# posgraph/coupe.optical_flow_based_deep_video_stabilization

Hardware: AMD Instinct MI355X
Metric: stabilised frame-pairs/sec @512x512 (higher is better)
Workload: dtype f32; 1 GPU; batch=8 512x512x27 frame stacks per GPU: FlowNetS-pyramid forward (5 flows) + flow resize/scale + tf_warp at 512x512; batch_per_gpu=8, height=512, width=512, cin=27, all_gather=False, vgg16_trunk=False, st_warp=none, plan_flags=0, plan_batch=0, full=False

## Files before the change

### coupe/optical_flow_based_deep_video_stabilization_amd/_lib.py

```python
from __future__ import annotations

import ctypes as C
import os

from . import build as _build

c_float_p = C.POINTER(C.c_float)
c_int32_p = C.POINTER(C.c_int32)


class VstabTensor(C.Structure):
    _fields_ = [("name", C.c_char_p), ("data", c_float_p), ("ndim", C.c_int32), ("shape", C.c_int32 * 4)]


class VstabWsEntry(C.Structure):
    _fields_ = [("name", C.c_char * 24), ("offset_bytes", C.c_int64), ("n", C.c_int32), ("h", C.c_int32),
                ("w", C.c_int32), ("c", C.c_int32), ("c_stride", C.c_int32)]


EXPORTS = {
    "vstab_create": (C.c_int, [C.POINTER(C.c_void_p), C.c_int]),
    "vstab_destroy": (None, [C.c_void_p]),
    "vstab_last_error": (C.c_char_p, [C.c_void_p]),
    "vstab_version": (C.c_char_p, []),
    "vstab_load_weights": (C.c_int, [C.c_void_p, C.POINTER(VstabTensor), C.c_int]),
    "vstab_workspace_bytes": (C.c_size_t, [C.c_int] * 4),
    "vstab_workspace_layout": (C.c_int, [C.c_int] * 4 + [C.POINTER(VstabWsEntry), C.c_int]),
    "vstab_workspace_layout_ctx": (C.c_int, [C.c_void_p] + [C.c_int] * 4 + [C.POINTER(VstabWsEntry), C.c_int]),
    "vstab_set_plan_batch": (C.c_int, [C.c_void_p, C.c_int]),
    "vstab_set_plan_flags": (C.c_int, [C.c_void_p, C.c_uint]),
    "vstab_workspace_bytes_ctx": (C.c_size_t, [C.c_void_p] + [C.c_int] * 4),
    "vstab_flownets_forward": (C.c_int, [C.c_void_p, C.c_void_p] + [C.c_int] * 4 + [C.c_void_p] * 5 +
                               [C.c_void_p, C.c_size_t, C.c_void_p]),
    "vstab_flow_resize_scale": (C.c_int, [C.c_void_p] + [C.c_int] * 3 + [C.c_void_p] + [C.c_int] * 4 + [C.c_void_p]),
    "vstab_resize_bilinear": (C.c_int, [C.c_void_p] + [C.c_int] * 4 + [C.c_void_p] + [C.c_int] * 2 + [C.c_void_p]),
    "vstab_resize_bilinear_slice3": (C.c_int, [C.c_void_p] + [C.c_int] * 5 + [C.c_void_p] + [C.c_int] * 2 + [C.c_void_p]),
    "vstab_warp_flow": (C.c_int, [C.c_void_p] * 3 + [C.c_int] * 4 + [C.c_void_p]),
    "vstab_selftest_div_const": (C.c_int, [C.c_float, C.c_uint, C.c_ulonglong, C.c_void_p, C.c_void_p]),
    "vstab_flow_glue_warp": (C.c_int, [C.c_void_p] + [C.c_int] * 3 + [C.c_void_p] * 3 + [C.c_int] * 5 + [C.c_void_p]),
    "vstab_stabilise_originalsize": (C.c_int, [C.c_void_p, C.c_void_p] + [C.c_int] * 4 + [C.c_void_p] + [C.c_int] * 2 + [C.c_void_p] * 8 +
                                     [C.c_size_t, C.c_void_p]),
    "vstab_trace_ranges": (C.c_int, [C.c_int]),
    "vstab_hbm_profile_enable": (C.c_int, [C.c_int]),
    "vstab_hbm_profile_read": (C.c_int, [C.c_int, C.POINTER(C.c_double), C.POINTER(C.c_int), C.POINTER(C.c_double)]),
    "vstab_get_pixel_value": (C.c_int, [C.c_void_p] * 4 + [C.c_int] * 6 + [C.c_void_p]),
# ... 144 lines not shown
```

### coupe/optical_flow_based_deep_video_stabilization_amd/build.py

```python
from __future__ import annotations

import os
import shutil
import subprocess

HERE = os.path.dirname(os.path.abspath(__file__))
CSRC = os.path.join(HERE, "csrc")
LIB = os.path.join(HERE, "libvstab_hip.so")
SOURCES = ("conv_mfma.hip", "conv_rowwin.hip", "conv_skinny.hip", "tap_panel.hip", "wino_gemm_stream.hip", "flow_ops.hip", "sampler_ops.hip", "sampler3d_ops.hip", "nldf_ops.hip", "clip_ops.hip", "train_ops.hip", "wgrad_mfma.hip", "winograd_ops.hip", "homography_ops.hip", "pack.cpp", "conv_desc.cpp", "api.cpp", "flownet_plan.cpp", "flownet_forward.cpp", "vgg_api.cpp", "nldf_api.cpp", "train_api.cpp")
HEADERS = ("vstab_internal.h", "api_internal.h", "conv_desc.h", "flownet_plan.h", "hbm_profile.h", "tile3.h", "st_axis.h", "conv_kloop_gfx950.inc", os.path.join("..", "..", "..", "include", "vstab.h"))
FLAGS = ["--offload-arch=gfx950", "-O3", "-std=c++17", "-ffp-contract=off", "-fPIC", "-fvisibility=hidden",
         "-Wall", "-Wno-unused-result"]


def hipcc() -> str:
    for c in (os.environ.get("HIPCC"), shutil.which("hipcc"), "/opt/rocm/bin/hipcc"):
        if c and os.path.exists(c):
            return c
    raise RuntimeError("hipcc not found (set HIPCC)")


STAMP = os.path.join(HERE, "libvstab_hip.so.srchash")


# ... 100 lines not shown
```

### coupe/optical_flow_based_deep_video_stabilization_amd/csrc/api.cpp

```cpp
#include <cmath>
#include <cstdlib>
#include <new>
#include <vector>

#include "api_internal.h"

using namespace vstab;

static thread_local std::string g_last_error;

int fail(vstab_ctx *ctx, int code, const char *fmt, ...)
{
    char buf[512];
    va_list ap;
    va_start(ap, fmt);
    vsnprintf(buf, sizeof buf, fmt, ap);
    va_end(ap);
    g_last_error = buf;
    if (ctx) { std::lock_guard<std::mutex> g(ctx->err_mu); ctx->err = buf; }
    return code;
}

void adopt_last_error(vstab_ctx *ctx)
{
// ... 58 lines not shown

extern "C" const char *vstab_version(void) { return "vstab-hip 0.1 (gfx950)"; }

extern "C" const char *vstab_last_error(const vstab_ctx *ctx) { return ctx ? ctx->err.c_str() : g_last_error.c_str(); }

extern "C" int vstab_create(vstab_ctx **out, int device)
{
    if (!out) return fail(nullptr, VSTAB_E_STATE, "vstab_create: out is NULL");
    *out = nullptr;
    int n = 0;
    HIP_TRY(nullptr, hipGetDeviceCount(&n));
    if (device < 0 || device >= n) return fail(nullptr, VSTAB_E_HIP, "vstab_create: device %d of %d", device, n);
    HIP_TRY(nullptr, hipSetDevice(device));
    HIP_TRY(nullptr, conv_set_attributes());
    HIP_TRY(nullptr, rowwin_set_attributes());
    HIP_TRY(nullptr, tap_panel_set_attributes());
    HIP_TRY(nullptr, wino_gemm_stream_set_attributes());
    vstab_ctx *c = new (std::nothrow) vstab_ctx();
    if (!c) return fail(nullptr, VSTAB_E_NOMEM, "vstab_create: out of host memory");
    c->device = device;
    *out = c;
    return VSTAB_OK;
}

extern "C" void vstab_destroy(vstab_ctx *ctx)
{
    if (!ctx) return;
    if (ctx->dev_weights) (void)hipFree(ctx->dev_weights);
    for (hipEvent_t e : ctx->prof_ev) (void)hipEventDestroy(e);
    if (ctx->vgg_weights) (void)hipFree(ctx->vgg_weights);
// ... 560 lines not shown
```

### coupe/optical_flow_based_deep_video_stabilization_amd/csrc/api_internal.h

```cpp
#pragma once
#include <cstdarg>
#include <cstdio>
#include <cstring>
#include <initializer_list>
#include <mutex>
#include <string>
#include <vector>

#include "../../../include/vstab.h"
#include "vstab_internal.h"

struct vstab_ctx {
    int device = 0;
    bool loaded = false;
    int cin = 0;
    std::string err;
    std::mutex err_mu;
    float *dev_weights = nullptr;
    size_t dev_weight_floats = 0;
    size_t enc_w[10], enc_b[10];
    size_t enc0_rw = 0;
    size_t zero_b = 0;
    size_t wino_w[10] = {0};
    size_t dec_w[4], dec_b[4];
    size_t wdec_w[4] = {0};
    size_t pred_w[4], pred_b[4];
    size_t tab_wp, tab_b, pred2_b;
    vstab::UpflowW up[4];
    int plan_batch = 0;
    unsigned plan_flags = 0;
    bool prof = false;
    std::vector<hipEvent_t> prof_ev;
    int prof_forwards = 0;
    double prof_flops[15] = {0};
    double prof_flops_direct[15] = {0};
    const char *prof_kernel[15] = {nullptr};
// ... 50 lines not shown
```

### coupe/optical_flow_based_deep_video_stabilization_amd/csrc/flownet_forward.cpp

```cpp
#include <cmath>
#include <cstdlib>

#include "flownet_plan.h"

using namespace vstab;

static const char *UP_NAME[4] = {"upsample6_5", "upsample5_4", "upsample4_3", "upsample3_2"};

extern "C" int vstab_load_weights(vstab_ctx *ctx, const vstab_tensor *t, int count)
{
    if (!ctx) return fail(nullptr, VSTAB_E_STATE, "vstab_load_weights: ctx is NULL");
    if (!t || count <= 0) return fail(ctx, VSTAB_E_WEIGHTS, "vstab_load_weights: no tensors");
    const vstab_tensor *w1 = find(t, count, "1/W_conv2d");
    if (!w1 || w1->ndim != 4) return fail(ctx, VSTAB_E_WEIGHTS, "missing variable 1/W_conv2d");
    const int cin = w1->shape[2];
    if (cin < 1 || cin > 4096) return fail(ctx, VSTAB_E_WEIGHTS, "1/W_conv2d: bad Cin %d", cin);

    std::vector<float> host;
    auto reserve = [&](size_t n) { size_t o = (host.size() + 63) / 64 * 64; host.resize(o + n, 0.f); return o; };
    std::vector<double> scale;
    auto need = [&](const std::string &name, std::initializer_list<int> s) -> const vstab_tensor * {
        const vstab_tensor *x = find(t, count, name);
        return shape_is(x, s) ? x : nullptr;
    };
// ... 14 lines not shown
        const int npad = padded_cols(e.cout);
        const KLayout L = conv_layout(e.k, e.k, ci, cs_in);
        scale.assign(npad, 1.0);
        ctx->enc_b[i] = reserve(npad);
        fold_bn(b->data, beta->data, mean->data, var->data, e.cout, npad, scale.data(), host.data() + ctx->enc_b[i]);
        ctx->enc_w[i] = reserve((size_t)L.ktiles() * npad * 32);
        pack_conv(W->data, scale.data(), e.k, e.k, ci, cs_in, e.cout, npad, L, host.data() + ctx->enc_w[i]);
        if (e.k == 3 && e.s == 1 && (ci & 31) == 0 && (e.cout & 127) == 0) {
            ctx->wino_w[i] = reserve((size_t)16 * (ci / 32) * e.cout * 32);
            pack_winograd(W->data, scale.data(), ci, e.cout, e.cout, host.data() + ctx->wino_w[i]);
        }
        if (i == 0) {
            const int lead = rowwin_lead(-e.p, cin), segp = rowwin_segp(-e.p, e.k, cin);
            ctx->enc0_rw = reserve((size_t)e.k * (segp / 32) * npad * 32);
            pack_conv_rowwin(W->data, scale.data(), e.k, e.k, cin, e.cout, npad, lead, segp, host.data() + ctx->enc0_rw);
        }
    }
    for (int l = 0; l < 4; ++l) {
        const Layer &d = dec_layer(l);
        const std::string n = d.name;
        const int co = d.cout, ci = d.cin, cs = in_buf(d).cs;
        NEED(W, n + "/W_deconv2d", 4, 4, co, ci)
        NEED(b, n + "/b_deconv2d", co)
        NEED(beta, n + "_bn/beta", co)
        NEED(mean, n + "_bn/moving_mean", co)
        NEED(var, n + "_bn/moving_variance", co)
        const int npad = padded_cols(co);
        scale.assign(npad, 1.0);
        ctx->dec_b[l] = reserve(npad);
        fold_bn(b->data, beta->data, mean->data, var->data, co, npad, scale.data(), host.data() + ctx->dec_b[l]);
// ... 85 lines not shown
        }
        const int rc = forward_chunk(ctx, feats + (size_t)b0 * H * W * Cin, bc, H, W, Cin,
                                     pf6 + (size_t)b0 * eh[9] * ew[9] * 2, pf5 + (size_t)b0 * eh[7] * ew[7] * 2,
                                     pf4 + (size_t)b0 * eh[5] * ew[5] * 2, pf3 + (size_t)b0 * eh[3] * ew[3] * 2,
                                     pf2 + (size_t)b0 * (H - 2) * (W - 2) * 2, workspace, workspace_bytes, stream_, (tail && all_fused) ? &t : nullptr);
        if (rc != VSTAB_OK) return rc;
        if (tail && all_fused && !t.fused) {
            if (b0 != 0) return fail(ctx, VSTAB_E_ALIGN, "stabilise: chunk %d of the batch misses the fused tail's alignment", b0 / chunk);
            all_fused = false;
        }
    }
    if (tail) tail->fused = all_fused;
    return VSTAB_OK;
}

static int forward_chunk(vstab_ctx *ctx, const float *feats, int B, int H, int W, int Cin, float *pf6, float *pf5,
                         float *pf4, float *pf3, float *pf2, void *workspace, size_t workspace_bytes, void *stream_, FusedTail *tail)
{
    Plan pl;
    const PlanPin pin = pin_of(ctx);
    if (!make_plan(B, H, W, Cin, pl, &pin)) return fail(ctx, VSTAB_E_SHAPE, "forward: unsupported problem %dx%dx%dx%d", B, H, W, Cin);
    if (workspace_bytes < pl.total) return fail(ctx, VSTAB_E_NOMEM, "forward: workspace %zu < %zu bytes", workspace_bytes, pl.total);
    if (((uintptr_t)workspace & 255) != 0) return fail(ctx, VSTAB_E_ALIGN, "forward: workspace must be 256-byte aligned");
    if (((uintptr_t)feats & 15) || ((uintptr_t)pf6 & 7) || ((uintptr_t)pf5 & 7) || ((uintptr_t)pf4 & 7) ||
        ((uintptr_t)pf3 & 7) || ((uintptr_t)pf2 & 7))
        return fail(ctx, VSTAB_E_ALIGN, "forward: feats must be 16-byte and flows 8-byte aligned");
    hipStream_t stream = (hipStream_t)stream_;
    char *ws = (char *)workspace;
    auto buf = [&](int b) { return (float *)(ws + pl.off[b]); };
    const float *dw = ctx->dev_weights;
// ... 27 lines not shown
            if (i >= 10 && i < 14 && pl.wdec[i - 10]) dmac = (double)B * p.Ho * p.Wo * 4.0 * NET[i].cin * p.N;
            ctx->prof_flops_direct[i] += 2.0 * dmac;
        }
    }
#define PROF_NAME(slot, name) do { if (ev) ctx->prof_kernel[slot] = (name); } while (0)
#define EV_A(slot) (ev ? ev[2 * (slot)] : nullptr)
#define EV_B(slot) (ev ? ev[2 * (slot) + 1] : nullptr)

    static const char *const HEAD_RANGE[4] = {"predict_flow6+upsample6_5", "predict_flow5+upsample5_4", "predict_flow4+upsample4_3", "predict_flow3+upsample3_2"};
    TraceRange whole_range("flownetS_pyramid");
    for (int i = 0; i < 10; ++i) {
        const Layer &e = NET[i];
        TraceRange layer_range(e.name);
        ConvParams p = pl.cp[i];
        if (i == 0) {
            RowWinParams r{};
            r.in = feats; r.out = buf(B_CONV1); r.wpk = dw + ctx->enc0_rw; r.bias = dw + ctx->enc_b[0];
            const long long in_bytes = (long long)B * H * W * Cin * 4;
            r.in_bytes = (unsigned)std::min<long long>(in_bytes, 0xFFFFFFFFLL);
            r.B = B; r.Hi = H; r.Wi = W; r.Cs_in = Cin; r.KH = e.k;
            r.SEGP = rowwin_segp(-e.p, e.k, Cin);
            r.s_in = e.s; r.off_y = -e.p;
            r.e_off = -e.p * Cin - rowwin_lead(-e.p, Cin);
            r.w_a = ((r.e_off % 4) + 4) % 4;
            r.MB = rowwin_mb(B, p.Ho, p.Wo);
            r.WLEN = round_up(r.s_in * Cin * (64 * r.MB - 1) + r.w_a + r.SEGP, 4);
            r.Ho = p.Ho; r.Wo = p.Wo; r.Cs_out = p.Cs_out; r.c_off = 0; r.N = p.N; r.Npad = p.Npad; r.act = 1;
            if (in_bytes < 0x80000000LL && rowwin_applicable(r)) {
                if (!tickets_cleared) { r.clear_words = tickets; r.clear_n = SKINNY_MAX_TILES; tickets_cleared = true; }
                const int rem = p.Wo % 128;
                if (r.MB == 2 && p.Wo > 128 && rem >= 1 && rem <= 64) {
                    RowWinParams t = r;
                    r.ntile_x = p.Wo / 128;
                    t.MB = 1; t.ox_base = r.ntile_x * 128; t.ntile_x = 1; t.clear_n = 0;
                    t.WLEN = round_up(t.s_in * Cin * 63 + t.w_a + t.SEGP, 4);
                    if (rowwin_applicable(t)) {
                        HIP_TRY(ctx, launch_conv_rowwin(r, stream, EV_A(0), nullptr));
                        HIP_TRY(ctx, launch_conv_rowwin(t, stream, nullptr, EV_B(0)));
                        PROF_NAME(0, "conv_rowwin_kernel<7, 2> + <4, 1> tail");
                        continue;
                    }
                    r.ntile_x = 0;
                }
                HIP_TRY(ctx, launch_conv_rowwin(r, stream, EV_A(0), EV_B(0)));
                PROF_NAME(0, r.MB == 2 ? "conv_rowwin_kernel<7, 2>" : "conv_rowwin_kernel<4, 1>");
                continue;
            }
        }
        if (!tickets_cleared) { HIP_TRY(ctx, hipMemsetAsync(tickets, 0, pl.bytes[B_TICKETS], stream)); tickets_cleared = true; }
        if (pl.wino[i]) {
            ConvParams q = pl.wcp[i];
            const int cin_i = e.cin;
            HIP_TRY(ctx, launch_wino_input(buf(e.in), B, pl.eh[i], pl.ew[i], in_buf(e).cs, 0, cin_i, buf(B_WINO_V), stream));
            q.in = buf(B_WINO_V); q.out = buf(B_WINO_M);
            q.wpk = dw + ctx->wino_w[i]; q.bias = dw + ctx->zero_b; q.partial = buf(B_PARTIAL);
            const int T_i = ((pl.eh[i] + 1) / 2) * ((pl.ew[i] + 1) / 2);
            const int P_i = wino_gemm_stream_positions(B, T_i, cin_i, e.cout);
            if (P_i > 0) {
                HIP_TRY(ctx, launch_wino_gemm_stream(q.in, q.wpk, q.out, B, T_i, cin_i, e.cout, P_i, stream, EV_A(i), EV_B(i)));
                PROF_NAME(i, "wino_gemm_stream_kernel");
            } else {
                HIP_TRY(ctx, launch_conv(q, pl.wtile[i], true, stream, EV_A(i), EV_B(i)));
// ... 236 lines not shown
```

### coupe/optical_flow_based_deep_video_stabilization_amd/csrc/flownet_plan.cpp

```cpp
#include <cmath>
#include <cstdlib>
#include <memory>
#include <new>

#include "flownet_plan.h"

using namespace vstab;

bool level_sizes(int H, int W, int *eh, int *ew)
{
    int h = H, w = W;
    for (int i = 0; i < 10; ++i) {
        h = (h + 2 * NET[i].p - NET[i].k) / NET[i].s + 1;
        w = (w + 2 * NET[i].p - NET[i].k) / NET[i].s + 1;
        if (h < 1 || w < 1) return false;
        eh[i] = h; ew[i] = w;
    }
    for (int l = 0; l < 4; ++l)
        if ((eh[LVL_ENC[l + 1]] + 1) / 2 != eh[LVL_ENC[l]] || (ew[LVL_ENC[l + 1]] + 1) / 2 != ew[LVL_ENC[l]]) return false;
    return H >= 3 && W >= 3;
}

static double split_cost_us(long long tiles, int KT, int ks, double slab_bytes, int BN, int BM, int *ks_eff_out)
{
// ... 153 lines not shown
        const Layer &e = NET[i];
        ConvParams &p = pl.cp[i];
        const int cin = i == 0 ? Cin : e.cin, cs_in = i == 0 ? Cin : in_buf(e).cs;
        p = conv_desc_plain(B, i == 0 ? H : pl.eh[i - 1], i == 0 ? W : pl.ew[i - 1], cin, cs_in, e.k, e.s, e.p, pl.eh[i], pl.ew[i], e.cout,
                            padded_cols(e.cout), out_buf(e).cs, e.c_off, 1);
        pl.tile[i] = default_tile(e.cout);
        pl.vec4[i] = (p.Cs_in % 4 == 0) && (p.SEG % 4 == 0);
        if (ref) { pl.tile[i] = ref->tile[i]; pl.skinny[i] = ref->skinny[i]; p.ksplit = ref->cp[i].ksplit; }
        else {
            pl.tile[i] = choose_tile_split(p, pl.tile[i], pl.vec4[i]);
            pl.skinny[i] = i > 0 && choose_skinny(p, pl.vec4[i], flags);
            if (pl.skinny[i]) pl.tile[i] = TILE_SKINNY;
        }
        if (p.ksplit > 1) partial_floats = std::max(partial_floats, (size_t)p.ksplit * p.Mmax * p.Npad);
    }
    size_t wino_v = 0, wino_m = 0;
    for (int i = 0; i < 10; ++i) {
        pl.wino[i] = false;
        const Layer &e = NET[i];
        if (e.k != 3 || e.s != 1 || e.p != 1 || pl.skinny[i]) continue;
        if (ref ? !ref->wino[i] : (in_buf(e).cs != e.cin || !wino_applies(B, pl.eh[i], pl.ew[i], e.cin, e.cout))) continue;
        const int TH = (pl.eh[i] + 1) / 2, TW = (pl.ew[i] + 1) / 2;
        pl.wcp[i] = conv_desc_wino_gemm(B, pl.eh[i], pl.ew[i], e.cin, e.cout);
        {
            const long long t128 = 16LL * ((pl.wcp[i].Mmax + 127) / 128) * (e.cout / 128);
            pl.wtile[i] = t128 >= 1024 ? TILE_128x128 : TILE_128x64;
        }
        wino_v = std::max(wino_v, (size_t)B * 16 * TH * TW * e.cin);
        wino_m = std::max(wino_m, (size_t)B * 16 * TH * TW * e.cout);
        pl.wino[i] = true;
// ... 87 lines not shown
    if (chunk < 1 || !make_plan(chunk, H, W, Cin, pl)) { fail(nullptr, VSTAB_E_SHAPE, "unsupported problem %dx%dx%dx%d", B, H, W, Cin); return 0; }
    return pl.total;
}

extern "C" int vstab_set_plan_batch(vstab_ctx *ctx, int batch)
{
    if (!ctx) return fail(nullptr, VSTAB_E_STATE, "set_plan_batch: ctx is NULL");
    if (batch < 0) return fail(ctx, VSTAB_E_SHAPE, "set_plan_batch: batch must be >= 0 (0 = plan for the batch of each call)");
    ctx->plan_batch = batch;
    return VSTAB_OK;
}

extern "C" int vstab_set_plan_flags(vstab_ctx *ctx, unsigned flags)
{
    if (!ctx) return fail(nullptr, VSTAB_E_STATE, "set_plan_flags: ctx is NULL");
    if (flags & ~(unsigned)(VSTAB_PLAN_NO_SKINNY | VSTAB_PLAN_NO_DUAL | VSTAB_PLAN_NO_TAIL | VSTAB_PLAN_NO_WDEC | VSTAB_PLAN_FORCE_WDEC)) return fail(ctx, VSTAB_E_SHAPE, "set_plan_flags: unknown flag bits 0x%x", flags);
    ctx->plan_flags = flags;
    return VSTAB_OK;
}

extern "C" size_t vstab_workspace_bytes_ctx(const vstab_ctx *ctx, int B, int H, int W, int Cin)
{
    Plan pl;
    const PlanPin pin = pin_of(ctx);
    if (pin.batch > 0 && B > pin.batch) { fail(nullptr, VSTAB_E_SHAPE, "batch %d exceeds the pinned plan batch %d", B, pin.batch); return 0; }
    const int chunk = B >= 1 ? chunk_size(pin, B, H, W, Cin) : 0;
    if (chunk < 1 || !make_plan(chunk, H, W, Cin, pl, &pin)) { fail(nullptr, VSTAB_E_SHAPE, "unsupported problem %dx%dx%dx%d", B, H, W, Cin); return 0; }
    return pl.total;
}

static int workspace_layout_of(const PlanPin *pin, int chunk, int H, int W, int Cin, vstab_ws_entry *entries, int max_entries)
// ... 116 lines not shown
```

### coupe/optical_flow_based_deep_video_stabilization_amd/csrc/flownet_plan.h

```cpp
#pragma once
#include "api_internal.h"
#include "conv_desc.h"

enum Buf { B_CONV1, B_CONCAT2, B_CONV3, B_CONCAT3, B_CONV4, B_CONCAT4, B_CONV5, B_CONCAT5, B_CONV6, B_CONV6_1, B_T,
           B_T6, B_T5, B_T4, B_T3, B_TICKETS, B_PARTIAL, B_WINO_V, B_WINO_M, N_BUF };
static_assert(B_PARTIAL == N_BUF - 3 && B_WINO_V == N_BUF - 2 && B_WINO_M == N_BUF - 1, "plan-dependent buffers must come last");

struct BufSpec { const char *name; int level, c, cs; };
constexpr BufSpec BUFS[N_BUF] = {
    {"conv1", 0, 64, 64},         {"concat2", 1, 194, 196},   {"conv3", 2, 256, 256},     {"concat3", 3, 386, 388},
    {"conv4", 4, 512, 512},       {"concat4", 5, 770, 772},   {"conv5", 6, 512, 512},     {"concat5", 7, 1026, 1028},
    {"conv6", 8, 1024, 1024},     {"conv6_1", 9, 1024, 1024}, {"pf2_taps", 1, 32, 32},    {"pf6_taps", 9, 32, 32},
    {"pf5_taps", 7, 32, 32},      {"pf4_taps", 5, 32, 32},    {"pf3_taps", 3, 32, 32},    {"tickets", -1, 0, 0},
    {"splitk", -1, 0, 0},         {"winograd_in", -1, 0, 0},  {"winograd_out", -1, 0, 0}};

enum LayerKind { L_CONV, L_DECONV, L_TAPS };
struct Layer { const char *name; LayerKind kind; int k, s, p, cin, cout, in, out, c_off; };
constexpr int N_LAYER = 19;
constexpr Layer NET[N_LAYER] = {
    {"conv1", L_CONV, 7, 2, 3, 0, 64, -1, B_CONV1, 0},              {"conv2", L_CONV, 5, 2, 2, 64, 128, B_CONV1, B_CONCAT2, 0},
    {"conv3", L_CONV, 5, 2, 2, 128, 256, B_CONCAT2, B_CONV3, 0},    {"conv3_1", L_CONV, 3, 1, 1, 256, 256, B_CONV3, B_CONCAT3, 0},
    {"conv4", L_CONV, 3, 2, 1, 256, 512, B_CONCAT3, B_CONV4, 0},    {"conv4_1", L_CONV, 3, 1, 1, 512, 512, B_CONV4, B_CONCAT4, 0},
    {"conv5", L_CONV, 3, 2, 1, 512, 512, B_CONCAT4, B_CONV5, 0},    {"conv5_1", L_CONV, 3, 1, 1, 512, 512, B_CONV5, B_CONCAT5, 0},
    {"conv6", L_CONV, 3, 2, 1, 512, 1024, B_CONCAT5, B_CONV6, 0},   {"conv6_1", L_CONV, 3, 1, 1, 1024, 1024, B_CONV6, B_CONV6_1, 0},
// ... 22 lines not shown
    for (int b = 0; b < N_BUF; ++b)
        if (BUFS[b].cs < BUFS[b].c || (BUFS[b].cs & 3)) return false;
    return NET[14].in == dec_layer(3).out;
}
static_assert(net_is_consistent(), "NET and BUFS disagree");

struct Plan {
    int B, H, W, Cin;
    int eh[10], ew[10];
    size_t off[N_BUF];
    size_t bytes[N_BUF];
    size_t total;
    vstab::ConvParams cp[N_LAYER];
    vstab::ConvTile tile[N_LAYER];
    bool vec4[N_LAYER];
    bool skinny[N_LAYER];
    bool wino[10];
    vstab::ConvParams wcp[10];
    vstab::ConvTile wtile[10];
    bool wdec[4];
    vstab::ConvParams wdcp[4];
    vstab::ConvTile wdtile[4];
    vstab::WdecGeom wdg[4];
    int buf_h(int b) const { return BUFS[b].level < 0 ? 0 : eh[BUFS[b].level]; }
    int buf_w(int b) const { return BUFS[b].level < 0 ? 0 : ew[BUFS[b].level]; }
};

struct PlanPin { int batch = 0; unsigned flags = 0; };
inline PlanPin pin_of(const vstab_ctx *ctx)
{
// ... 9 lines not shown
```

### coupe/optical_flow_based_deep_video_stabilization_amd/csrc/pack.cpp

```cpp
#include <cmath>
#include <cstring>

#include "vstab_internal.h"

namespace vstab {

KLayout klayout_run(int kh, int kw, int cs_in)
{
    KLayout L{kh, 1, kw * cs_in, round_up(kw * cs_in, 32), 0};
    return L;
}
KLayout klayout_tap(int kh, int kw, int cin, int cs_in)
{
    KLayout L{kh, kw, cin, round_up(cin, 32), cs_in};
    return L;
}
KLayout klayout_deconv(int cs_in) { return klayout_run(2, 2, cs_in); }

void fold_bn(const float *b, const float *beta, const float *mean, const float *var, int cout, int npad,
             double *scale, float *bias_out)
{
    for (int n = 0; n < npad; ++n) {
        double s = 1.0, bb = 0.0;
        if (n < cout) {
// ... 43 lines not shown
}

void pack_conv_rowwin(const float *W, const double *scale, int kh, int kw, int cin, int cout, int npad, int lead,
                      int segp, float *wpk)
{
    const int kpr = segp / 32;
    std::memset(wpk, 0, sizeof(float) * (size_t)kh * kpr * npad * 32);
    for (int ky = 0; ky < kh; ++ky)
        for (int kx = 0; kx < kw; ++kx)
            for (int ci = 0; ci < cin; ++ci) {
                const int k = lead + kx * cin + ci;
                float *row = wpk + ((size_t)ky * kpr + k / 32) * npad * 32;
                for (int n = 0; n < cout; ++n)
                    row[(size_t)n * 32 + perm_rowwin(k & 31)] =
                        (float)((double)W[(((size_t)ky * kw + kx) * cin + ci) * cout + n] * scale[n]);
            }
}

void pack_deconv(const float *W, const double *scale, int cin, int cs_in, int cout, int npad, float *wpk)
{
    const KLayout L = klayout_deconv(cs_in);
    const size_t phase_floats = (size_t)L.ktiles() * npad * 32;
    for (int py = 0; py < 2; ++py)
        for (int px = 0; px < 2; ++px) {
            pack_generic(L, cs_in, cin, 2, cout, npad,
                         [&](int t, int bx, int ci, int n) {
                             const int ky = 3 - py - 2 * t, kx = 3 - px - 2 * bx;
                             return (float)((double)W[(((size_t)ky * 4 + kx) * cout + n) * cin + ci] * scale[n]);
                         },
                         wpk + (size_t)(py * 2 + px) * phase_floats);
// ... 148 lines not shown
```

### coupe/optical_flow_based_deep_video_stabilization_amd/csrc/vstab_internal.h

```cpp
#pragma once
#include <hip/hip_runtime.h>
#include <stddef.h>
#include <stdint.h>

namespace vstab {

inline int round_up_c(int a, int b) { return (a + b - 1) / b * b; }

#ifdef __HIPCC__
#define VSTAB_HD __host__ __device__
#else
#define VSTAB_HD
#endif
VSTAB_HD inline void xcd_remap_calc(unsigned Nx, unsigned Ny, unsigned Nz, unsigned lin, unsigned &bx, unsigned &by, unsigned &bz)
{
    const unsigned T = Nx * Ny * Nz;
    const unsigned q = T >> 3, r = T & 7u, c = lin & 7u, idx = lin >> 3;
    const unsigned nl = (c < r ? c * (q + 1) : r * (q + 1) + (c - r) * q) + idx;
    unsigned t2;
    if ((Ny & (Ny - 1)) == 0) { const unsigned s = 31u - (unsigned)__builtin_clz(Ny); by = nl & (Ny - 1); t2 = nl >> s; }
    else { by = nl % Ny; t2 = nl / Ny; }
    if ((Nz & (Nz - 1)) == 0) { const unsigned s = 31u - (unsigned)__builtin_clz(Nz); bz = t2 & (Nz - 1); bx = t2 >> s; }
    else { bz = t2 % Nz; bx = t2 / Nz; }
}
// ... 131 lines not shown
    int asm_loop;
    int stream_rows;
    unsigned *clear_words;
    int clear_n;
    int ox_base, ntile_x;
};
inline int rowwin_mb(int B, int Ho, int Wo) { return (long long)B * Ho * ((Wo + 127) / 128) < 512 ? 1 : 2; }
bool rowwin_applicable(const RowWinParams &p);
hipError_t rowwin_set_attributes();
hipError_t launch_conv_rowwin(const RowWinParams &p, hipStream_t stream, hipEvent_t ev_start = nullptr,
                              hipEvent_t ev_stop = nullptr);
inline int rowwin_lead(int off_x, int cs) { return ((off_x * cs) % 2 != 0) ? 1 : 0; }
inline int rowwin_segp(int off_x, int kw, int cs) { return round_up_c(rowwin_lead(off_x, cs) + kw * cs, 32); }
void pack_conv_rowwin(const float *W, const double *scale, int kh, int kw, int cin, int cout, int npad,
                      int lead, int segp, float *wpk);

hipError_t launch_wino_outgrad(const float *dy, int B, int H, int W, int Cs, int c_off, int C, float *dM, hipStream_t stream);
hipError_t launch_wino_filter_grad(const float *dU, int cin, int cout, float *dW, hipStream_t stream);
int wino_gemm_stream_positions(int B, int T, int cin, int cout);
hipError_t launch_wino_gemm_stream(const float *V, const float *wpk, float *M, int B, int T, int cin, int cout, int P, hipStream_t stream,
                                   hipEvent_t ev_start = nullptr, hipEvent_t ev_stop = nullptr);
hipError_t wino_gemm_stream_set_attributes();
hipError_t launch_wino_input(const float *x, int B, int H, int W, int Cs, int c_off, int C, float *V, hipStream_t stream,
                             bool pos_major = false);
hipError_t launch_wino_weights(const float *W, int cin, int cout, int transpose, float *Wt, hipStream_t stream);
hipError_t launch_wino_output(const float *M, int B, int Ho, int Wo, int C, const float *bias, int act, float *out, int Cs_out, int c_off,
                              hipStream_t stream);

struct WdecGeom {
    int NTy, NTx;
// ... 260 lines not shown
```

### include/vstab.h

```cpp
#ifndef VSTAB_H
#define VSTAB_H

#include <stddef.h>
#include <stdint.h>

#ifdef __cplusplus
extern "C" {
#endif

#define VSTAB_OK          0
#define VSTAB_E_SHAPE    -1
#define VSTAB_E_ALIGN    -2
#define VSTAB_E_HIP      -3
#define VSTAB_E_NOMEM    -4
#define VSTAB_E_WEIGHTS  -5
#define VSTAB_E_STATE    -6

#if defined(__GNUC__)
#define VSTAB_API __attribute__((visibility("default")))
#else
#define VSTAB_API
#endif

typedef struct vstab_ctx vstab_ctx;
// ... 202 lines not shown
VSTAB_API int vstab_flow_mean_fill(const float *flow, int B, int h, int w, float *out, void *stream);

VSTAB_API size_t vstab_homography_workspace_bytes(int B, int H, int W, int K);
VSTAB_API int vstab_homography_fit(const float *flow, int B, int H, int W, int K, unsigned seed, double thresh, int refine,
                                   int stride, double *Hout, int32_t *inliers, void *workspace, size_t workspace_bytes,
                                   void *stream);
VSTAB_API int vstab_warp_perspective_u8(const uint8_t *src, int B, int sh, int sw, const double *Hm, uint8_t *dst, int oh, int ow,
                                        void *stream);


#define VSTAB_PLAN_NO_SKINNY 1u
#define VSTAB_PLAN_NO_DUAL 2u
#define VSTAB_PLAN_NO_TAIL 4u
#define VSTAB_PLAN_NO_WDEC 8u
#define VSTAB_PLAN_FORCE_WDEC 16u
VSTAB_API int vstab_set_plan_flags(vstab_ctx *ctx, unsigned flags);

VSTAB_API int vstab_profile_enable(vstab_ctx *ctx, int enable);
VSTAB_API int vstab_profile_reset(vstab_ctx *ctx);
VSTAB_API int vstab_profile_read(vstab_ctx *ctx, double *ms_sum15, double *flops15, int *n_forwards);
VSTAB_API int vstab_profile_read_direct(vstab_ctx *ctx, double *flops15);
VSTAB_API int vstab_profile_kernel_name(vstab_ctx *ctx, int slot, char *buf, int cap);

VSTAB_API int vstab_selftest_div_const(float d, unsigned first_bits, unsigned long long count, unsigned long long *bad_count_dev,
                                       void *stream);

VSTAB_API int vstab_trace_ranges(int on);

VSTAB_API int vstab_hbm_profile_enable(int mode);
VSTAB_API int vstab_hbm_profile_read(int slot, double *ms_sum, int *launches, double *alg_bytes_sum);

// ... 17 lines not shown
```

Baseline: 2850 frame-pairs/s.

## Run conv1 on bf16 MFMA with three-way split for fp32-level accuracy

Adds a new conv1 row-window kernel that splits fp32 inputs and weights into three bf16 components (hi/mid/lo) and computes the product with six bf16 MFMA passes, replacing the fp32 rowwin path when cout is 64. The input split is done in LDS per kernel row, and weights are pre-split at load time. The aim is to use the much higher bf16 matrix throughput for the first, large-spatial convolution while keeping accuracy close to fp32. It adds split arithmetic, three times the LDS planes and extra MFMA passes, and it can be turned off with a new plan flag.

```diff
diff --git a/coupe/optical_flow_based_deep_video_stabilization_amd/_lib.py b/coupe/optical_flow_based_deep_video_stabilization_amd/_lib.py
--- a/coupe/optical_flow_based_deep_video_stabilization_amd/_lib.py
+++ b/coupe/optical_flow_based_deep_video_stabilization_amd/_lib.py
@@ -29,6 +29,7 @@
     "vstab_workspace_layout_ctx": (C.c_int, [C.c_void_p] + [C.c_int] * 4 + [C.POINTER(VstabWsEntry), C.c_int]),
     "vstab_set_plan_batch": (C.c_int, [C.c_void_p, C.c_int]),
     "vstab_set_plan_flags": (C.c_int, [C.c_void_p, C.c_uint]),
+    "vstab_conv1_forward": (C.c_int, [C.c_void_p, C.c_void_p] + [C.c_int] * 4 + [C.c_void_p, C.c_int, C.c_int, C.c_void_p]),
     "vstab_workspace_bytes_ctx": (C.c_size_t, [C.c_void_p] + [C.c_int] * 4),
     "vstab_flownets_forward": (C.c_int, [C.c_void_p, C.c_void_p] + [C.c_int] * 4 + [C.c_void_p] * 5 +
                                [C.c_void_p, C.c_size_t, C.c_void_p]),
diff --git a/coupe/optical_flow_based_deep_video_stabilization_amd/build.py b/coupe/optical_flow_based_deep_video_stabilization_amd/build.py
--- a/coupe/optical_flow_based_deep_video_stabilization_amd/build.py
+++ b/coupe/optical_flow_based_deep_video_stabilization_amd/build.py
@@ -7,7 +7,7 @@
 HERE = os.path.dirname(os.path.abspath(__file__))
 CSRC = os.path.join(HERE, "csrc")
 LIB = os.path.join(HERE, "libvstab_hip.so")
-SOURCES = ("conv_mfma.hip", "conv_rowwin.hip", "conv_skinny.hip", "tap_panel.hip", "wino_gemm_stream.hip", "flow_ops.hip", "sampler_ops.hip", "sampler3d_ops.hip", "nldf_ops.hip", "clip_ops.hip", "train_ops.hip", "wgrad_mfma.hip", "winograd_ops.hip", "homography_ops.hip", "pack.cpp", "conv_desc.cpp", "api.cpp", "flownet_plan.cpp", "flownet_forward.cpp", "vgg_api.cpp", "nldf_api.cpp", "train_api.cpp")
+SOURCES = ("conv_mfma.hip", "conv_rowwin.hip", "conv1_bf16x3.hip", "conv_skinny.hip", "tap_panel.hip", "wino_gemm_stream.hip", "flow_ops.hip", "sampler_ops.hip", "sampler3d_ops.hip", "nldf_ops.hip", "clip_ops.hip", "train_ops.hip", "wgrad_mfma.hip", "winograd_ops.hip", "homography_ops.hip", "pack.cpp", "conv_desc.cpp", "api.cpp", "flownet_plan.cpp", "flownet_forward.cpp", "vgg_api.cpp", "nldf_api.cpp", "train_api.cpp")
 HEADERS = ("vstab_internal.h", "api_internal.h", "conv_desc.h", "flownet_plan.h", "hbm_profile.h", "tile3.h", "st_axis.h", "conv_kloop_gfx950.inc", os.path.join("..", "..", "..", "include", "vstab.h"))
 FLAGS = ["--offload-arch=gfx950", "-O3", "-std=c++17", "-ffp-contract=off", "-fPIC", "-fvisibility=hidden",
          "-Wall", "-Wno-unused-result"]
diff --git a/coupe/optical_flow_based_deep_video_stabilization_amd/csrc/api.cpp b/coupe/optical_flow_based_deep_video_stabilization_amd/csrc/api.cpp
--- a/coupe/optical_flow_based_deep_video_stabilization_amd/csrc/api.cpp
+++ b/coupe/optical_flow_based_deep_video_stabilization_amd/csrc/api.cpp
@@ -96,6 +96,7 @@
     HIP_TRY(nullptr, hipSetDevice(device));
     HIP_TRY(nullptr, conv_set_attributes());
     HIP_TRY(nullptr, rowwin_set_attributes());
+    HIP_TRY(nullptr, conv1_bf16x3_set_attributes());
     HIP_TRY(nullptr, tap_panel_set_attributes());
     HIP_TRY(nullptr, wino_gemm_stream_set_attributes());
     vstab_ctx *c = new (std::nothrow) vstab_ctx();
diff --git a/coupe/optical_flow_based_deep_video_stabilization_amd/csrc/api_internal.h b/coupe/optical_flow_based_deep_video_stabilization_amd/csrc/api_internal.h
--- a/coupe/optical_flow_based_deep_video_stabilization_amd/csrc/api_internal.h
+++ b/coupe/optical_flow_based_deep_video_stabilization_amd/csrc/api_internal.h
@@ -20,6 +20,7 @@
     size_t dev_weight_floats = 0;
     size_t enc_w[10], enc_b[10];
     size_t enc0_rw = 0;
+    size_t enc0_b3 = 0;
     size_t zero_b = 0;
     size_t wino_w[10] = {0};
     size_t dec_w[4], dec_b[4];
diff --git a/coupe/optical_flow_based_deep_video_stabilization_amd/csrc/conv1_bf16x3.hip b/coupe/optical_flow_based_deep_video_stabilization_amd/csrc/conv1_bf16x3.hip
--- /dev/null
+++ b/coupe/optical_flow_based_deep_video_stabilization_amd/csrc/conv1_bf16x3.hip
@@ -0,0 +1,220 @@
+#include <hip/hip_ext.h>
+
+#include "vstab_internal.h"
+
+namespace vstab {
+
+typedef float f32x4 __attribute__((ext_vector_type(4)));
+typedef float f32x16 __attribute__((ext_vector_type(16)));
+typedef unsigned u32x2 __attribute__((ext_vector_type(2)));
+typedef unsigned u32x4 __attribute__((ext_vector_type(4)));
+typedef __bf16 bf16x4 __attribute__((ext_vector_type(4)));
+typedef __bf16 bf16x8 __attribute__((ext_vector_type(8)));
+
+template <int NWIN4, int MB>
+__global__ __launch_bounds__(256) void conv1_bf16x3_kernel(const RowWinParams p)
+{
+    extern __shared__ __attribute__((aligned(16))) char smem[];
+    unsigned *planes = reinterpret_cast<unsigned *>(smem);
+
+    const int tid = threadIdx.x, lane = tid & 63, wave = tid >> 6;
+    const int wm = wave >> 1, wn = wave & 1;
+    const int li = lane & 31, lh = lane >> 5;
+    unsigned bx_, by_, bz_;
+    xcd_remap(bx_, by_, bz_);
+    if (p.clear_n > 0 && blockIdx.x == 0 && blockIdx.y == 0 && blockIdx.z == 0)
+        for (int i = tid; i < p.clear_n; i += 256) p.clear_words[i] = 0u;
+    const int oy = (int)bx_;
+    const int ox0 = p.ox_base + (int)by_ * (64 * MB), n = (int)bz_;
+    const int pix_step = p.s_in * p.Cs_in;
+    const int row_floats = p.Wi * p.Cs_in;
+    const int g0 = pix_step * ox0 + p.e_off - p.w_a;
+
+    const __amdgpu_buffer_rsrc_t rin = __builtin_amdgcn_make_buffer_rsrc(const_cast<float *>(p.in), 0, p.in_bytes, 0x00020000);
+    const unsigned OOB = 0xC0000000u;
+
+    f32x4 wv[NWIN4];
+    auto load_window = [&](int ky) {
+        const int iy = oy * p.s_in + p.off_y + ky;
+        const bool yok = (unsigned)iy < (unsigned)p.Hi;
+        const int rowbase = ((n * p.Hi + iy) * p.Wi) * p.Cs_in;
+#pragma unroll
+        for (int j = 0; j < NWIN4; ++j) {
+            const int c4 = tid + 256 * j;
+            const int g = g0 + 4 * c4;
+            const bool ok = yok && g >= 0 && g < row_floats && 4 * c4 < p.WLEN;
+            const unsigned off = ok ? (unsigned)(rowbase + g) * 4u : OOB;
+            wv[j] = __builtin_bit_cast(f32x4, __builtin_amdgcn_raw_buffer_load_b128(rin, off, 0, 0));
+        }
+    };
+    const int plane_w = p.WLEN >> 1;
+    auto split_store = [&]() {
+#pragma unroll
+        for (int j = 0; j < NWIN4; ++j) {
+            const int c4 = tid + 256 * j;
+            if (4 * c4 < p.WLEN) {
+                bf16x4 h, m, l;
+#pragma unroll
+                for (int e = 0; e < 4; ++e) {
+                    const float x = wv[j][e];
+                    h[e] = (__bf16)x;
+                    const float r1 = x - (float)h[e];
+                    m[e] = (__bf16)r1;
+                    const float r2 = r1 - (float)m[e];
+                    l[e] = (__bf16)r2;
+                }
+                *reinterpret_cast<u32x2 *>(planes + 2 * c4) = __builtin_bit_cast(u32x2, h);
+                *reinterpret_cast<u32x2 *>(planes + plane_w + 2 * c4) = __builtin_bit_cast(u32x2, m);
+                *reinterpret_cast<u32x2 *>(planes + 2 * plane_w + 2 * c4) = __builtin_bit_cast(u32x2, l);
+            }
+        }
+    };
+
+    const int KG = p.SEGP >> 4;
+    const int NG = p.KH * KG;
+    const unsigned *bbase = reinterpret_cast<const unsigned *>(p.wpk) + (wn * 32 + li) * 8 + lh * 4;
+    auto load_b = [&](u32x4 (&b)[3], int G) {
+        const unsigned *s = bbase + (long long)(G < NG ? G : NG - 1) * (3 * 512);
+#pragma unroll
+        for (int q = 0; q < 3; ++q) b[q] = *reinterpret_cast<const u32x4 *>(s + q * 512);
+    };
+    const int a_w0 = (pix_step * (wm * 32 * MB + li) + p.w_a + 8 * lh) >> 1;
+    const int a_w1 = a_w0 + ((pix_step * 32) >> 1);
+    auto load_a = [&](u32x4 (&a)[3 * MB], int g) {
+#pragma unroll
+        for (int mb = 0; mb < MB; ++mb)
+#pragma unroll
+            for (int q = 0; q < 3; ++q) {
+                const unsigned *s = planes + q * plane_w + (mb ? a_w1 : a_w0) + 8 * g;
+                u32x4 v;
+                v.x = s[0]; v.y = s[1]; v.z = s[2]; v.w = s[3];
+                a[mb * 3 + q] = v;
+            }
+    };
+
+    f32x16 acc[MB];
+#pragma unroll
+    for (int a = 0; a < MB; ++a)
+#pragma unroll
+        for (int r = 0; r < 16; ++r) acc[a][r] = 0.f;
+
+    auto mma = [&](const u32x4 (&a)[3 * MB], const u32x4 (&b)[3]) {
+        constexpr int PA[6] = {2, 1, 0, 1, 0, 0}, PB[6] = {0, 1, 2, 0, 1, 0};
+#pragma unroll
+        for (int t = 0; t < 6; ++t)
+#pragma unroll
+            for (int mb = 0; mb < MB; ++mb)
+                acc[mb] = __builtin_amdgcn_mfma_f32_32x32x16_bf16(__builtin_bit_cast(bf16x8, a[mb * 3 + PA[t]]),
+                                                                  __builtin_bit_cast(bf16x8, b[PB[t]]), acc[mb], 0, 0, 0);
+    };
+
+    u32x4 a0[3 * MB], a1[3 * MB], b0[3], b1[3];
+    load_window(0);
+    load_b(b0, 0);
+    split_store();
+    __syncthreads();
+    int G = 0;
+    for (int ky = 0; ky < p.KH; ++ky) {
+        const bool more = ky + 1 < p.KH;
+        if (more) load_window(ky + 1);
+        load_a(a0, 0);
+        __builtin_amdgcn_sched_barrier(0);
+        for (int g = 0; g < KG; g += 2, G += 2) {
+            load_a(a1, g + 1);
+            load_b(b1, G + 1);
+            __builtin_amdgcn_sched_barrier(0);
+            mma(a0, b0);
+            __builtin_amdgcn_sched_barrier(0);
+            if (g + 2 < KG) load_a(a0, g + 2);
+            load_b(b0, G + 2);
+            __builtin_amdgcn_sched_barrier(0);
+            mma(a1, b1);
+            __builtin_amdgcn_sched_barrier(0);
+        }
+        if (more) {
+            __syncthreads();
+            split_store();
+            __syncthreads();
+        }
+    }
+
+    const int col = wn * 32 + li;
+    if (p.out_vec4) {
+        constexpr int TP = 64 * MB;
+        __syncthreads();
+        float *sC = reinterpret_cast<float *>(smem);
+        const float bv = col < p.N ? p.bias[col] : 0.f;
+#pragma unroll
+        for (int mb = 0; mb < MB; ++mb)
+#pragma unroll
+            for (int r = 0; r < 16; ++r) sC[(wm * 32 * MB + mb * 32 + (r & 3) + 8 * (r >> 2) + 4 * lh) * 64 + col] = acc[mb][r] + bv;
+        __syncthreads();
+        const float slope = p.act == 1 ? 0.1f : 0.0f;
+        float *orow = p.out + ((long long)(n * p.Ho + oy) * p.Wo + ox0) * p.Cs_out + p.c_off;
+#pragma unroll 4
+        for (int e = tid; e < TP * 16; e += 256) {
+            const int px = e >> 4, c4 = (e & 15) * 4;
+            if (ox0 + px >= p.Wo || c4 >= p.N) continue;
+            f32x4 v = *reinterpret_cast<const f32x4 *>(sC + px * 64 + c4);
+            if (p.act) {
+#pragma unroll
+                for (int i = 0; i < 4; ++i) v[i] = fmaxf(v[i], slope * v[i]);
+            }
+            float *o = orow + (long long)px * p.Cs_out + c4;
+            if (c4 + 4 <= p.N) *reinterpret_cast<f32x4 *>(o) = v;
+            else for (int i = 0; c4 + i < p.N; ++i) o[i] = v[i];
+        }
+    } else if (col < p.N) {
+        const float bv = p.bias[col];
+#pragma unroll
+        for (int mb = 0; mb < MB; ++mb)
+#pragma unroll
+            for (int r = 0; r < 16; ++r) {
+                const int ox = ox0 + wm * 32 * MB + mb * 32 + (r & 3) + 8 * (r >> 2) + 4 * lh;
+                if (ox < p.Wo) {
+                    float v = acc[mb][r] + bv;
+                    if (p.act) v = fmaxf(v, (p.act == 1 ? 0.1f : 0.0f) * v);
+                    p.out[((long long)(n * p.Ho + oy) * p.Wo + ox) * p.Cs_out + p.c_off + col] = v;
+                }
+            }
+    }
+}
+
+bool conv1_bf16x3_applicable(const RowWinParams &p)
+{
+    return rowwin_applicable(p) && p.KH >= 1 && (p.SEGP % 32) == 0 && p.SEGP >= 32;
+}
+
+hipError_t conv1_bf16x3_set_attributes()
+{
+    const hipError_t e = hipFuncSetAttribute(reinterpret_cast<const void *>(conv1_bf16x3_kernel<7, 2>),
+                                             hipFuncAttributeMaxDynamicSharedMemorySize, 3 * 7 * 1024 * 2);
+    if (e != hipSuccess) return e;
+    return hipFuncSetAttribute(reinterpret_cast<const void *>(conv1_bf16x3_kernel<4, 1>),
+                               hipFuncAttributeMaxDynamicSharedMemorySize, 3 * 4 * 1024 * 2);
+}
+
+hipError_t launch_conv1_bf16x3(const RowWinParams &p, hipStream_t stream, hipEvent_t ev_start, hipEvent_t ev_stop)
+{
+    if (!conv1_bf16x3_applicable(p)) return hipErrorInvalidValue;
+    const int tile = 64 * p.MB;
+    if (p.ox_base < 0 || p.ox_base >= p.Wo || (p.ox_base & 1) || p.ntile_x < 0) return hipErrorInvalidValue;
+    const int ntx = p.ntile_x > 0 ? p.ntile_x : (p.Wo - p.ox_base + tile - 1) / tile;
+    dim3 grid(p.Ho, ntx, p.B), block(256);
+    RowWinParams q = p;
+    const size_t lds = (size_t)3 * p.WLEN * 2;
+    q.out_vec4 = (((uintptr_t)p.out & 15) == 0 && (p.Cs_out & 3) == 0 && (p.c_off & 3) == 0 && lds >= (size_t)tile * 64 * 4) ? 1 : 0;
+    q.asm_loop = 0;
+    q.stream_rows = 0;
+    const bool timed = ev_start || ev_stop;
+    if (p.MB == 2) {
+        if (timed) hipExtLaunchKernelGGL((conv1_bf16x3_kernel<7, 2>), grid, block, lds, stream, ev_start, ev_stop, 0, q);
+        else conv1_bf16x3_kernel<7, 2><<<grid, block, lds, stream>>>(q);
+    } else {
+        if (timed) hipExtLaunchKernelGGL((conv1_bf16x3_kernel<4, 1>), grid, block, lds, stream, ev_start, ev_stop, 0, q);
+        else conv1_bf16x3_kernel<4, 1><<<grid, block, lds, stream>>>(q);
+    }
+    return hipGetLastError();
+}
+
+}
diff --git a/coupe/optical_flow_based_deep_video_stabilization_amd/csrc/flownet_forward.cpp b/coupe/optical_flow_based_deep_video_stabilization_amd/csrc/flownet_forward.cpp
--- a/coupe/optical_flow_based_deep_video_stabilization_amd/csrc/flownet_forward.cpp
+++ b/coupe/optical_flow_based_deep_video_stabilization_amd/csrc/flownet_forward.cpp
@@ -1,5 +1,6 @@
 #include <cmath>
 #include <cstdlib>
+#include <memory>
 
 #include "flownet_plan.h"
 
@@ -52,6 +53,11 @@
             const int lead = rowwin_lead(-e.p, cin), segp = rowwin_segp(-e.p, e.k, cin);
             ctx->enc0_rw = reserve((size_t)e.k * (segp / 32) * npad * 32);
             pack_conv_rowwin(W->data, scale.data(), e.k, e.k, cin, e.cout, npad, lead, segp, host.data() + ctx->enc0_rw);
+            ctx->enc0_b3 = 0;
+            if (npad == 64) {
+                ctx->enc0_b3 = reserve((size_t)e.k * (segp / 16) * 3 * 64 * 16 / 2);
+                pack_conv1_bf16x3(W->data, scale.data(), e.k, e.k, cin, e.cout, lead, segp, reinterpret_cast<uint16_t *>(host.data() + ctx->enc0_b3));
+            }
         }
     }
     for (int l = 0; l < 4; ++l) {
@@ -167,6 +173,77 @@
     return VSTAB_OK;
 }
 
+static int conv1_rowwin(vstab_ctx *ctx, bool bf16x3, const float *feats, int B, int H, int W, int Cin, int Ho, int Wo, int N, int Npad,
+                        float *out, int cs_out, int c_off, unsigned *tickets, hipStream_t stream, hipEvent_t ev_a, hipEvent_t ev_b,
+                        const char **kname, bool *launched)
+{
+    const Layer &e = NET[0];
+    const float *dw = ctx->dev_weights;
+    *launched = false;
+    RowWinParams r{};
+    r.in = feats; r.out = out; r.wpk = dw + ctx->enc0_rw; r.bias = dw + ctx->enc_b[0];
+    const long long in_bytes = (long long)B * H * W * Cin * 4;
+    r.in_bytes = (unsigned)std::min<long long>(in_bytes, 0xFFFFFFFFLL);
+    r.B = B; r.Hi = H; r.Wi = W; r.Cs_in = Cin; r.KH = e.k;
+    r.SEGP = rowwin_segp(-e.p, e.k, Cin);
+    r.s_in = e.s; r.off_y = -e.p;
+    r.e_off = -e.p * Cin - rowwin_lead(-e.p, Cin);
+    r.w_a = ((r.e_off % 4) + 4) % 4;
+    r.MB = rowwin_mb(B, Ho, Wo);
+    r.WLEN = round_up(r.s_in * Cin * (64 * r.MB - 1) + r.w_a + r.SEGP, 4);
+    r.Ho = Ho; r.Wo = Wo; r.Cs_out = cs_out; r.c_off = c_off; r.N = N; r.Npad = Npad; r.act = 1;
+    if (in_bytes >= 0x80000000LL || !rowwin_applicable(r)) return VSTAB_OK;
+    const bool b3 = bf16x3 && ctx->enc0_b3 != 0 && conv1_bf16x3_applicable(r);
+    if (b3) r.wpk = dw + ctx->enc0_b3;
+    auto launch1 = [&](const RowWinParams &q, hipEvent_t a, hipEvent_t b) {
+        return b3 ? launch_conv1_bf16x3(q, stream, a, b) : launch_conv_rowwin(q, stream, a, b);
+    };
+    if (tickets) { r.clear_words = tickets; r.clear_n = SKINNY_MAX_TILES; }
+    *launched = true;
+    const int rem = Wo % 128;
+    if (r.MB == 2 && Wo > 128 && rem >= 1 && rem <= 64) {
+        RowWinParams t = r;
+        r.ntile_x = Wo / 128;
+        t.MB = 1; t.ox_base = r.ntile_x * 128; t.ntile_x = 1; t.clear_n = 0;
+        t.WLEN = round_up(t.s_in * Cin * 63 + t.w_a + t.SEGP, 4);
+        if (rowwin_applicable(t)) {
+            HIP_TRY(ctx, launch1(r, ev_a, nullptr));
+            HIP_TRY(ctx, launch1(t, nullptr, ev_b));
+            *kname = b3 ? "conv1_bf16x3_kernel<7, 2> + <4, 1> tail" : "conv_rowwin_kernel<7, 2> + <4, 1> tail";
+            return VSTAB_OK;
+        }
+        r.ntile_x = 0;
+    }
+    HIP_TRY(ctx, launch1(r, ev_a, ev_b));
+    if (b3) *kname = r.MB == 2 ? "conv1_bf16x3_kernel<7, 2>" : "conv1_bf16x3_kernel<4, 1>";
+    else *kname = r.MB == 2 ? "conv_rowwin_kernel<7, 2>" : "conv_rowwin_kernel<4, 1>";
+    return VSTAB_OK;
+}
+
+extern "C" int vstab_conv1_forward(vstab_ctx *ctx, const float *feats, int B, int H, int W, int Cin, float *out, int cs_out, int c_off,
+                                   void *stream_)
+{
+    if (!ctx) return fail(nullptr, VSTAB_E_STATE, "conv1_forward: ctx is NULL");
+    if (!ctx->loaded) return fail(ctx, VSTAB_E_STATE, "conv1_forward: vstab_load_weights has not been called");
+    if (Cin != ctx->cin) return fail(ctx, VSTAB_E_SHAPE, "conv1_forward: feats has %d channels, weights expect %d", Cin, ctx->cin);
+    if (!feats || !out) return fail(ctx, VSTAB_E_STATE, "conv1_forward: NULL buffer");
+    const PlanPin pin = pin_of(ctx);
+    std::unique_ptr<Plan> pl(new (std::nothrow) Plan);
+    if (!pl) return fail(ctx, VSTAB_E_NOMEM, "conv1_forward: out of host memory");
+    if (B < 1 || !make_plan(B, H, W, Cin, *pl, &pin)) return fail(ctx, VSTAB_E_SHAPE, "conv1_forward: unsupported problem %dx%dx%dx%d", B, H, W, Cin);
+    const ConvParams &p = pl->cp[0];
+    if (c_off < 0 || cs_out < c_off + p.N || (long long)B * p.Ho * p.Wo * cs_out * 4 >= 0x80000000LL)
+        return fail(ctx, VSTAB_E_SHAPE, "conv1_forward: output slice %d + %d of %d channels", c_off, p.N, cs_out);
+    if (((uintptr_t)feats & 15) || ((uintptr_t)out & 3)) return fail(ctx, VSTAB_E_ALIGN, "conv1_forward: feats must be 16-byte aligned");
+    const char *kname = nullptr;
+    bool launched = false;
+    const int rc = conv1_rowwin(ctx, pl->conv1_bf16x3, feats, B, H, W, Cin, p.Ho, p.Wo, p.N, p.Npad, out, cs_out, c_off, nullptr,
+                                (hipStream_t)stream_, nullptr, nullptr, &kname, &launched);
+    if (rc != VSTAB_OK) return rc;
+    if (!launched) return fail(ctx, VSTAB_E_SHAPE, "conv1_forward: the row-window kernels do not take this geometry");
+    return VSTAB_OK;
+}
+
 static int forward_chunk(vstab_ctx *ctx, const float *feats, int B, int H, int W, int Cin, float *pf6, float *pf5,
                          float *pf4, float *pf3, float *pf2, void *workspace, size_t workspace_bytes, void *stream_, FusedTail *tail)
 {
@@ -224,38 +301,12 @@
         TraceRange layer_range(e.name);
         ConvParams p = pl.cp[i];
         if (i == 0) {
-            RowWinParams r{};
-            r.in = feats; r.out = buf(B_CONV1); r.wpk = dw + ctx->enc0_rw; r.bias = dw + ctx->enc_b[0];
-            const long long in_bytes = (long long)B * H * W * Cin * 4;
-            r.in_bytes = (unsigned)std::min<long long>(in_bytes, 0xFFFFFFFFLL);
-            r.B = B; r.Hi = H; r.Wi = W; r.Cs_in = Cin; r.KH = e.k;
-            r.SEGP = rowwin_segp(-e.p, e.k, Cin);
-            r.s_in = e.s; r.off_y = -e.p;
-            r.e_off = -e.p * Cin - rowwin_lead(-e.p, Cin);
-            r.w_a = ((r.e_off % 4) + 4) % 4;
-            r.MB = rowwin_mb(B, p.Ho, p.Wo);
-            r.WLEN = round_up(r.s_in * Cin * (64 * r.MB - 1) + r.w_a + r.SEGP, 4);
-            r.Ho = p.Ho; r.Wo = p.Wo; r.Cs_out = p.Cs_out; r.c_off = 0; r.N = p.N; r.Npad = p.Npad; r.act = 1;
-            if (in_bytes < 0x80000000LL && rowwin_applicable(r)) {
-                if (!tickets_cleared) { r.clear_words = tickets; r.clear_n = SKINNY_MAX_TILES; tickets_cleared = true; }
-                const int rem = p.Wo % 128;
-                if (r.MB == 2 && p.Wo > 128 && rem >= 1 && rem <= 64) {
-                    RowWinParams t = r;
-                    r.ntile_x = p.Wo / 128;
-                    t.MB = 1; t.ox_base = r.ntile_x * 128; t.ntile_x = 1; t.clear_n = 0;
-                    t.WLEN = round_up(t.s_in * Cin * 63 + t.w_a + t.SEGP, 4);
-                    if (rowwin_applicable(t)) {
-                        HIP_TRY(ctx, launch_conv_rowwin(r, stream, EV_A(0), nullptr));
-                        HIP_TRY(ctx, launch_conv_rowwin(t, stream, nullptr, EV_B(0)));
-                        PROF_NAME(0, "conv_rowwin_kernel<7, 2> + <4, 1> tail");
-                        continue;
-                    }
-                    r.ntile_x = 0;
-                }
-                HIP_TRY(ctx, launch_conv_rowwin(r, stream, EV_A(0), EV_B(0)));
-                PROF_NAME(0, r.MB == 2 ? "conv_rowwin_kernel<7, 2>" : "conv_rowwin_kernel<4, 1>");
-                continue;
-            }
+            const char *kname = nullptr;
+            bool launched = false;
+            const int rc = conv1_rowwin(ctx, pl.conv1_bf16x3, feats, B, H, W, Cin, p.Ho, p.Wo, p.N, p.Npad, buf(B_CONV1), p.Cs_out, 0,
+                                        tickets_cleared ? nullptr : tickets, stream, EV_A(0), EV_B(0), &kname, &launched);
+            if (rc != VSTAB_OK) return rc;
+            if (launched) { tickets_cleared = true; PROF_NAME(0, kname); continue; }
         }
         if (!tickets_cleared) { HIP_TRY(ctx, hipMemsetAsync(tickets, 0, pl.bytes[B_TICKETS], stream)); tickets_cleared = true; }
         if (pl.wino[i]) {
diff --git a/coupe/optical_flow_based_deep_video_stabilization_amd/csrc/flownet_plan.cpp b/coupe/optical_flow_based_deep_video_stabilization_amd/csrc/flownet_plan.cpp
--- a/coupe/optical_flow_based_deep_video_stabilization_amd/csrc/flownet_plan.cpp
+++ b/coupe/optical_flow_based_deep_video_stabilization_amd/csrc/flownet_plan.cpp
@@ -191,6 +191,8 @@
         }
         if (p.ksplit > 1) partial_floats = std::max(partial_floats, (size_t)p.ksplit * p.Mmax * p.Npad);
     }
+    pl.conv1_bf16x3 = ref ? ref->conv1_bf16x3
+                          : (!(flags & VSTAB_PLAN_CONV1_FP32) && NET[0].cout == 64 && rowwin_segp(-NET[0].p, NET[0].k, Cin) <= 192);
     size_t wino_v = 0, wino_m = 0;
     for (int i = 0; i < 10; ++i) {
         pl.wino[i] = false;
@@ -308,7 +310,7 @@
 extern "C" int vstab_set_plan_flags(vstab_ctx *ctx, unsigned flags)
 {
     if (!ctx) return fail(nullptr, VSTAB_E_STATE, "set_plan_flags: ctx is NULL");
-    if (flags & ~(unsigned)(VSTAB_PLAN_NO_SKINNY | VSTAB_PLAN_NO_DUAL | VSTAB_PLAN_NO_TAIL | VSTAB_PLAN_NO_WDEC | VSTAB_PLAN_FORCE_WDEC)) return fail(ctx, VSTAB_E_SHAPE, "set_plan_flags: unknown flag bits 0x%x", flags);
+    if (flags & ~(unsigned)(VSTAB_PLAN_NO_SKINNY | VSTAB_PLAN_NO_DUAL | VSTAB_PLAN_NO_TAIL | VSTAB_PLAN_NO_WDEC | VSTAB_PLAN_FORCE_WDEC | VSTAB_PLAN_CONV1_FP32)) return fail(ctx, VSTAB_E_SHAPE, "set_plan_flags: unknown flag bits 0x%x", flags);
     ctx->plan_flags = flags;
     return VSTAB_OK;
 }
diff --git a/coupe/optical_flow_based_deep_video_stabilization_amd/csrc/flownet_plan.h b/coupe/optical_flow_based_deep_video_stabilization_amd/csrc/flownet_plan.h
--- a/coupe/optical_flow_based_deep_video_stabilization_amd/csrc/flownet_plan.h
+++ b/coupe/optical_flow_based_deep_video_stabilization_amd/csrc/flownet_plan.h
@@ -60,6 +60,7 @@
     vstab::ConvParams cp[N_LAYER];
     vstab::ConvTile tile[N_LAYER];
     bool vec4[N_LAYER];
+    bool conv1_bf16x3;
     bool skinny[N_LAYER];
     bool wino[10];
     vstab::ConvParams wcp[10];
diff --git a/coupe/optical_flow_based_deep_video_stabilization_amd/csrc/pack.cpp b/coupe/optical_flow_based_deep_video_stabilization_amd/csrc/pack.cpp
--- a/coupe/optical_flow_based_deep_video_stabilization_amd/csrc/pack.cpp
+++ b/coupe/optical_flow_based_deep_video_stabilization_amd/csrc/pack.cpp
@@ -81,6 +81,43 @@
                 for (int n = 0; n < cout; ++n)
                     row[(size_t)n * 32 + perm_rowwin(k & 31)] =
                         (float)((double)W[(((size_t)ky * kw + kx) * cin + ci) * cout + n] * scale[n]);
+            }
+}
+
+static inline uint16_t bf16_rne(float x)
+{
+    uint32_t u;
+    std::memcpy(&u, &x, 4);
+    if ((u & 0x7fffffffu) > 0x7f800000u) return (uint16_t)((u >> 16) | 0x40u);
+    return (uint16_t)((u + 0x7fffu + ((u >> 16) & 1u)) >> 16);
+}
+static inline float bf16_float(uint16_t b)
+{
+    const uint32_t u = (uint32_t)b << 16;
+    float x;
+    std::memcpy(&x, &u, 4);
+    return x;
+}
+
+void pack_conv1_bf16x3(const float *W, const double *scale, int kh, int kw, int cin, int cout, int lead, int segp, uint16_t *wpk)
+{
+    const int kg = segp / 16;
+    std::memset(wpk, 0, sizeof(uint16_t) * (size_t)kh * kg * 3 * 64 * 16);
+    for (int ky = 0; ky < kh; ++ky)
+        for (int kx = 0; kx < kw; ++kx)
+            for (int ci = 0; ci < cin; ++ci) {
+                const int k = lead + kx * cin + ci;
+                uint16_t *grp = wpk + ((size_t)ky * kg + k / 16) * 3 * 64 * 16;
+                for (int n = 0; n < cout && n < 64; ++n) {
+                    const float w = (float)((double)W[(((size_t)ky * kw + kx) * cin + ci) * cout + n] * scale[n]);
+                    const uint16_t h = bf16_rne(w);
+                    const float r1 = w - bf16_float(h);
+                    const uint16_t m = bf16_rne(r1);
+                    const float r2 = r1 - bf16_float(m);
+                    const uint16_t l = bf16_rne(r2);
+                    const size_t at = (size_t)n * 16 + (k & 15);
+                    grp[at] = h; grp[64 * 16 + at] = m; grp[2 * 64 * 16 + at] = l;
+                }
             }
 }
 
diff --git a/coupe/optical_flow_based_deep_video_stabilization_amd/csrc/vstab_internal.h b/coupe/optical_flow_based_deep_video_stabilization_amd/csrc/vstab_internal.h
--- a/coupe/optical_flow_based_deep_video_stabilization_amd/csrc/vstab_internal.h
+++ b/coupe/optical_flow_based_deep_video_stabilization_amd/csrc/vstab_internal.h
@@ -169,6 +169,12 @@
 inline int rowwin_segp(int off_x, int kw, int cs) { return round_up_c(rowwin_lead(off_x, cs) + kw * cs, 32); }
 void pack_conv_rowwin(const float *W, const double *scale, int kh, int kw, int cin, int cout, int npad,
                       int lead, int segp, float *wpk);
+
+bool conv1_bf16x3_applicable(const RowWinParams &p);
+hipError_t conv1_bf16x3_set_attributes();
+hipError_t launch_conv1_bf16x3(const RowWinParams &p, hipStream_t stream, hipEvent_t ev_start = nullptr,
+                               hipEvent_t ev_stop = nullptr);
+void pack_conv1_bf16x3(const float *W, const double *scale, int kh, int kw, int cin, int cout, int lead, int segp, uint16_t *wpk);
 
 hipError_t launch_wino_outgrad(const float *dy, int B, int H, int W, int Cs, int c_off, int C, float *dM, hipStream_t stream);
 hipError_t launch_wino_filter_grad(const float *dU, int cin, int cout, float *dW, hipStream_t stream);
diff --git a/include/vstab.h b/include/vstab.h
--- a/include/vstab.h
+++ b/include/vstab.h
@@ -240,7 +240,11 @@
 #define VSTAB_PLAN_NO_TAIL 4u
 #define VSTAB_PLAN_NO_WDEC 8u
 #define VSTAB_PLAN_FORCE_WDEC 16u
+#define VSTAB_PLAN_CONV1_FP32 32u
 VSTAB_API int vstab_set_plan_flags(vstab_ctx *ctx, unsigned flags);
+
+VSTAB_API int vstab_conv1_forward(vstab_ctx *ctx, const float *feats, int B, int H, int W, int Cin, float *out, int cs_out, int c_off,
+                                  void *stream);
 
 VSTAB_API int vstab_profile_enable(vstab_ctx *ctx, int enable);
 VSTAB_API int vstab_profile_reset(vstab_ctx *ctx);
```

New measurement: 3020 frame-pairs/s (median of 6 runs). +6.0%, better.
